# yuanqing-wang/stag

Hardware: AMD Instinct MI355X
Metric: aggregated edges/sec, stochastic-aggregation layer-forward, ogbn-arxiv-shaped CSR (higher is better)
Workload: dtype f32

## Files before the change

stag_amd/csrc/agg_plain.hpp:

```cpp
#pragma once
#include "agg_kernel.hpp"

namespace stag {

#ifndef STAG_PLAIN_WAVES
#define STAG_PLAIN_WAVES 7
#endif

typedef float f32x2_t __attribute__((ext_vector_type(2)));

template <int KIND, bool RELU>
__device__ __forceinline__ void plain_draw4(uint32_t c0, uint32_t c1, const PhiloxKey& key, f32x2_t p0, float p1,
                                            f32x2_t (&w)[2]) {
  uint32_t r[4];
  philox4x32_10(c0, c1, key, r);
  const f32x2_t s = {p1, p1};
  if constexpr (KIND == kNormal) {
    const f32x2_t z01 = f32x2_t{bm_cos(r[1]), bm_sin(r[1])} * bm_radius(r[0]);
    const f32x2_t z23 = f32x2_t{bm_cos(r[3]), bm_sin(r[3])} * bm_radius(r[2]);
    w[0] = __builtin_elementwise_fma(s, z01, p0);
    w[1] = __builtin_elementwise_fma(s, z23, p0);
  } else if constexpr (KIND == kUniform) {
    w[0] = __builtin_elementwise_fma(s, f32x2_t{u01(r[0]), u01(r[1])}, p0);
    w[1] = __builtin_elementwise_fma(s, f32x2_t{u01(r[2]), u01(r[3])}, p0);
  } else {
    w[0] = f32x2_t{u01(r[0]) < p0.x ? 1.0f : 0.0f, u01(r[1]) < p0.y ? 1.0f : 0.0f};
    w[1] = f32x2_t{u01(r[2]) < p0.x ? 1.0f : 0.0f, u01(r[3]) < p0.y ? 1.0f : 0.0f};
  }
  if constexpr (RELU) {
    w[0] = __builtin_elementwise_max(w[0], f32x2_t{0.f, 0.f});
    w[1] = __builtin_elementwise_max(w[1], f32x2_t{0.f, 0.f});
  }
}

template <int KIND, int LPE, bool RELU, class TEAM>
__device__ __forceinline__ void plain_walk(const AggArgs& a, TEAM& T, const int b, const int pend, const int len) {
  const __amdgpu_buffer_rsrc_t ri =
      __builtin_amdgcn_make_buffer_rsrc(const_cast<int32_t*>(a.indices), 0, (int)a.idx_bytes, 0x00020000);
  f32x2_t p0 = {a.p0s, a.p0s};
  asm volatile("" : "+v"(p0));
  const float p1 = KIND == kUniform ? a.p1s - a.p0s : a.p1s;
  const uint32_t pos1 = a.pos_lo + 1u;
  f32x2_t s01 = {0.f, 0.f}, s23 = {0.f, 0.f}, c01 = {0.f, 0.f}, c23 = {0.f, 0.f};
  const int pend1 = pend - 1;
  for (int p = b; p < pend; p += 2) {
    const bool two = p < pend1;
#if STAG_LOAD_PRIO
    __builtin_amdgcn_s_setprio(3);
#endif
    const int u0 = (int)__builtin_amdgcn_raw_buffer_load_b32(ri, p << 2, 0, 0);
    int u1;
    if (two) u1 = (int)__builtin_amdgcn_raw_buffer_load_b32(ri, (p << 2) + 4, 0, 0);
    uint32_t n0 = a.pos_lo + (uint32_t)p, n1 = pos1 + (uint32_t)p;
    asm volatile("" : "+v"(n0));
    asm volatile("" : "+v"(n1));
    u32x4_t x1;
    const u32x4_t x0 = __builtin_amdgcn_raw_buffer_load_b128(T.rx, (int)(__umul24((uint32_t)u0, a.ldxb) + T.koff), 0, STAG_X_AUX);
    if (two) x1 = __builtin_amdgcn_raw_buffer_load_b128(T.rx, (int)(__umul24((uint32_t)u1, a.ldxb) + T.koff), 0, STAG_X_AUX);
#if STAG_LOAD_PRIO
    if (len > STAG_PRIO_MIN_LEN) __builtin_amdgcn_s_setprio(2); else __builtin_amdgcn_s_setprio(0);
#endif
    f32x2_t w0[2], w1[2];
    plain_draw4<KIND, RELU>(n0, T.c1, T.key, p0, p1, w0);
    if (two) plain_draw4<KIND, RELU>(n1, T.c1, T.key, p0, p1, w1);
    const f32x2_t zero = {0.f, 0.f};
    f32x2_t t01 = __builtin_elementwise_fma(w0[0], f32x2_t{__uint_as_float(x0.x), __uint_as_float(x0.y)}, zero);
    f32x2_t t23 = __builtin_elementwise_fma(w0[1], f32x2_t{__uint_as_float(x0.z), __uint_as_float(x0.w)}, zero);
    if (two) {
      asm volatile("" ::: "memory");
      t01 = __builtin_elementwise_fma(w1[0], f32x2_t{__uint_as_float(x1.x), __uint_as_float(x1.y)}, t01);
      t23 = __builtin_elementwise_fma(w1[1], f32x2_t{__uint_as_float(x1.z), __uint_as_float(x1.w)}, t23);
    }
    if (T.kahan) {
      const f32x2_t y01 = t01 - c01, y23 = t23 - c23;
      const f32x2_t n01 = s01 + y01, n23 = s23 + y23;
      c01 = (n01 - s01) - y01; c23 = (n23 - s23) - y23;
      s01 = n01; s23 = n23;
    } else {
      s01 += t01; s23 += t23;
    }
  }
  T.acc[0] = s01.x; T.acc[1] = s01.y; T.acc[2] = s23.x; T.acc[3] = s23.y;
}

template <int KIND, int LPE, bool RELU, bool WALK>
__global__ __launch_bounds__(STAG_BLOCK_THREADS)
__attribute__((amdgpu_waves_per_eu(STAG_PLAIN_WAVES, STAG_PLAIN_WAVES))) void agg_plain_kernel(const AggArgs a_in) {
  static_assert(KIND >= kNormal && (LPE == 32 || LPE == 64), "the plain launch: sampled noise, 32 or 64 lanes per row");
  static_assert(heavy_slots_of<KIND, LPE>() == 1 && mult_of<KIND, LPE>() == 1, "wide shapes walk one slot, one block");
  AggArgs a = a_in;
  if constexpr (WALK) {
    STAG_PIN_S(a.walk.smask); STAG_PIN_S(a.walk.sshift); STAG_PIN_S(a.walk.jh_light);
    STAG_PIN_S(a.walk.sh); STAG_PIN_S(a.walk.lbase); STAG_PIN_S(a.walk.sl); STAG_PIN_S(a.walk.n_total);
  }
  STAG_PIN_S(a.D); STAG_PIN_S(a.units); STAG_PIN_S(a.indptr); STAG_PIN_S(a.indices);
  STAG_PIN_S(a.x); STAG_PIN_S(a.ldxb); STAG_PIN_S(a.x_bytes); STAG_PIN_S(a.idx_bytes);
  STAG_PIN_S(a.p0s); STAG_PIN_S(a.p1s);
  STAG_PIN_S(a.key.k0); STAG_PIN_S(a.key.k1); STAG_PIN_S(a.key.o0); STAG_PIN_S(a.key.o1); STAG_PIN_S(a.key.epoch);
  STAG_PIN_S(a.pos_lo); STAG_PIN_S(a.pos_hi); STAG_PIN_S(a.chunk_base);
  a.nflags = RELU ? kFlagRelu : 0;
  a.in_norm = 0; a.norm_scale_out = nullptr;
  a.src_scale = nullptr;
  a.nidx = nullptr; a.eid = nullptr;
  a.pmode = STAG_PARAM_SCALAR; a.p0 = nullptr; a.p1 = nullptr;
  a.wide = 0;
  __builtin_assume(a.x_bytes != 0);
  __builtin_assume(a.out != nullptr);

  const int c = threadIdx.x % LPE;
  constexpr int TPB = STAG_BLOCK_THREADS / LPE;
  if constexpr (!WALK) {
    const int unit = blockIdx.x * TPB + threadIdx.x / LPE;
    if (unit >= a.n_units) return;
    agg_unit<KIND, LPE, true, 0, 1, 1, 1, false, false, false, RELU ? 3 : 1>(a, unit, c, 0);
  } else {
    const AggArgs::Walk w = a.walk;
    const int stripe = blockIdx.x & w.smask;
    int j = blockIdx.x >> w.sshift;
    int unit0, end;
    if (j < w.jh_light) {
      unit0 = stripe * w.sh + j * TPB;
      end = (stripe + 1) * w.sh;
    } else {
      j -= w.jh_light;
      unit0 = w.lbase + stripe * w.sl + j * TPB;
      end = min(w.lbase + (stripe + 1) * w.sl, w.n_total);
    }
    const int unit = unit0 + threadIdx.x / LPE;
    if (unit >= end) return;
    agg_unit<KIND, LPE, true, 0, 1, 1, 1, false, false, true, RELU ? 3 : 1>(a, unit, c, 0);
  }
}

template <int KIND>
inline void agg_launch_plain_impl(const AggArgs& a, int lpe, bool walk, dim3 grid, hipStream_t s) {
  const dim3 block(STAG_BLOCK_THREADS);
  const bool relu = (a.nflags & kFlagRelu) != 0;
#define STAG_PLAIN_GO(L, R, W) hipLaunchKernelGGL((agg_plain_kernel<KIND, L, R, W>), grid, block, STAG_AGG_LDS_BYTES, s, a)
  if (lpe == 32) {
    if (walk) { if (relu) STAG_PLAIN_GO(32, true, true); else STAG_PLAIN_GO(32, false, true); }
    else      { if (relu) STAG_PLAIN_GO(32, true, false); else STAG_PLAIN_GO(32, false, false); }
  } else {
    if (walk) { if (relu) STAG_PLAIN_GO(64, true, true); else STAG_PLAIN_GO(64, false, true); }
    else      { if (relu) STAG_PLAIN_GO(64, true, false); else STAG_PLAIN_GO(64, false, false); }
  }
#undef STAG_PLAIN_GO
}

}
```

stag_amd/csrc/noise.hpp:

```cpp
#pragma once
#include <hip/hip_runtime.h>
#include <stdint.h>

namespace stag {

constexpr uint32_t kPhiloxM0 = 0xD2511F53u;
constexpr uint32_t kPhiloxM1 = 0xCD9E8D57u;
constexpr uint32_t kPhiloxW0 = 0x9E3779B9u;
constexpr uint32_t kPhiloxW1 = 0xBB67AE85u;

struct PhiloxKey {
  uint32_t k0, k1;
  uint32_t o0, o1;
  const uint64_t* epoch;
};

__device__ __forceinline__ PhiloxKey resolve_epoch(PhiloxKey k) {
  if (k.epoch) {
    const uint64_t o = (((uint64_t)k.o1 << 32) | k.o0) + *k.epoch;
    k.o0 = (uint32_t)o;
    k.o1 = (uint32_t)(o >> 32);
  }
  return k;
}

inline bool counter_space_ok(int64_t pos_base, int64_t n_edges, int64_t chunk_base, int64_t n_chunk) {
  return pos_base >= 0 && n_edges >= 0 && pos_base <= (1ll << 44) - n_edges && chunk_base >= 0 &&
         chunk_base + n_chunk <= (1ll << 20);
}

__device__ __forceinline__ PhiloxKey key_plus(PhiloxKey k, uint64_t d) {
  const uint64_t o = (((uint64_t)k.o1 << 32) | k.o0) + d;
  k.o0 = (uint32_t)o;
  k.o1 = (uint32_t)(o >> 32);
  return k;
}

__device__ __forceinline__ void philox4x32_10(uint32_t c0, uint32_t c1, const PhiloxKey& key,
                                              uint32_t (&r)[4]) {
  uint32_t c2 = key.o0, c3 = key.o1;
  uint32_t k0 = key.k0, k1 = key.k1;
#pragma unroll
  for (int i = 0; i < 10; ++i) {
    const uint64_t p0 = (uint64_t)kPhiloxM0 * c0;
    const uint64_t p1 = (uint64_t)kPhiloxM1 * c2;
    const uint32_t n0 = __builtin_amdgcn_bitop3_b32((uint32_t)(p1 >> 32), c1, k0, 0x96);
    const uint32_t n2 = __builtin_amdgcn_bitop3_b32((uint32_t)(p0 >> 32), c3, k1, 0x96);
    c1 = (uint32_t)p1;
    c3 = (uint32_t)p0;
    c0 = n0;
    c2 = n2;
    k0 += kPhiloxW0;
    k1 += kPhiloxW1;
  }
  r[0] = c0; r[1] = c1; r[2] = c2; r[3] = c3;
}

__device__ __forceinline__ void philox_at(int64_t gpos, uint32_t chunk, const PhiloxKey& key,
                                          uint32_t (&r)[4]) {
  const uint32_t c0 = (uint32_t)((uint64_t)gpos & 0xFFFFFFFFull);
  const uint32_t c1 = chunk | ((uint32_t)((uint64_t)gpos >> 32) << 20);
  philox4x32_10(c0, c1, key, r);
}

__device__ __forceinline__ uint32_t ctr1_of(int64_t gpos, uint32_t chunk) {
  return chunk | ((uint32_t)((uint64_t)gpos >> 32) << 20);
}

__device__ __forceinline__ float f12(uint32_t r) {
  return __uint_as_float((r & 0x007FFFFFu) | 0x3F800000u);
}

__device__ __forceinline__ float u01(uint32_t r) { return f12(r) - 1.0f; }

__device__ __forceinline__ float bm_radius(uint32_t ra) {
  const float u1 = 2.0f - f12(ra);
  return __builtin_amdgcn_sqrtf(-1.3862943611198906f * __builtin_amdgcn_logf(u1));
}
__device__ __forceinline__ float bm_cos(uint32_t rb) { return __builtin_amdgcn_cosf(f12(rb)); }
__device__ __forceinline__ float bm_sin(uint32_t rb) { return __builtin_amdgcn_sinf(f12(rb)); }

__device__ __forceinline__ void box_muller(uint32_t ra, uint32_t rb, float& za, float& zb) {
  const float rad = bm_radius(ra);
  za = rad * bm_cos(rb);
  zb = rad * bm_sin(rb);
}

enum : int { kNone = 0, kExplicit = 1, kNormal = 2, kUniform = 3, kBernoulli = 4 };

enum : int { kFlagRelu = 1, kDerivShift = 1, kDerivMask = 3, kFlagLogScale = 8 };

__device__ __forceinline__ float exp_scale(float log_scale) { return __expf(log_scale); }

template <int KIND>
__device__ __forceinline__ void draw4(uint32_t c0, uint32_t c1, const PhiloxKey& key,
                                      const float (&a)[4], const float (&b)[4], int flags,
                                      float (&w)[4]) {
  static_assert(KIND >= kNormal, "draw4 is for sampled noise");
  uint32_t r[4];
  philox4x32_10(c0, c1, key, r);
  float t[4];
  if constexpr (KIND == kNormal) {
    box_muller(r[0], r[1], t[0], t[1]);
    box_muller(r[2], r[3], t[2], t[3]);
#pragma unroll
    for (int j = 0; j < 4; ++j) w[j] = __builtin_fmaf(b[j], t[j], a[j]);
  } else if constexpr (KIND == kUniform) {
#pragma unroll
    for (int j = 0; j < 4; ++j) { t[j] = u01(r[j]); w[j] = __builtin_fmaf(b[j] - a[j], t[j], a[j]); }
  } else {
#pragma unroll
    for (int j = 0; j < 4; ++j) w[j] = u01(r[j]) < a[j] ? 1.0f : 0.0f;
  }
  const int deriv = (flags >> kDerivShift) & kDerivMask;
  if (deriv == 0) {
    if (flags & kFlagRelu) {
#pragma unroll
      for (int j = 0; j < 4; ++j) w[j] = fmaxf(w[j], 0.0f);
    }
    return;
  }
  if constexpr (KIND != kBernoulli) {
#pragma unroll
    for (int j = 0; j < 4; ++j) {
      const float mask = ((flags & kFlagRelu) && !(w[j] > 0.0f)) ? 0.0f : 1.0f;
      float d;
      if constexpr (KIND == kNormal)
        d = (deriv == 1) ? 1.0f : ((flags & kFlagLogScale) ? t[j] * b[j] : t[j]);
      else d = (deriv == 1) ? 1.0f - t[j] : t[j];
      w[j] = d * mask;
    }
  }
}

template <int KIND>
__device__ __forceinline__ void draw4_grad(uint32_t c0, uint32_t c1, const PhiloxKey& key,
                                           const float (&a)[4], const float (&b)[4], int flags,
                                           float (&w)[4], float (&d0)[4], float (&d1)[4]) {
  static_assert(KIND == kNormal || KIND == kUniform, "only reparameterised draws have derivatives");
  uint32_t r[4];
  philox4x32_10(c0, c1, key, r);
  float t[4];
  if constexpr (KIND == kNormal) {
    box_muller(r[0], r[1], t[0], t[1]);
    box_muller(r[2], r[3], t[2], t[3]);
#pragma unroll
    for (int j = 0; j < 4; ++j) w[j] = __builtin_fmaf(b[j], t[j], a[j]);
  } else {
#pragma unroll
    for (int j = 0; j < 4; ++j) { t[j] = u01(r[j]); w[j] = __builtin_fmaf(b[j] - a[j], t[j], a[j]); }
  }
#pragma unroll
  for (int j = 0; j < 4; ++j) {
    const float mask = ((flags & kFlagRelu) && !(w[j] > 0.0f)) ? 0.0f : 1.0f;
    if (flags & kFlagRelu) w[j] = fmaxf(w[j], 0.0f);
    d0[j] = ((KIND == kNormal) ? 1.0f : 1.0f - t[j]) * mask;
    d1[j] = (KIND == kNormal && (flags & kFlagLogScale)) ? t[j] * b[j] * mask : t[j] * mask;
  }
}

}
```

Measured before the change: 12.70 billion.

## Add wave-uniform walk with scalar index loads and split Philox rounds

Adds a wave-level walk path for 64-lane rows. The edge index and counter are made wave-uniform, so neighbour ids come from scalar constant loads and the gather offset moves to the scalar operand. Philox is split so that the first rounds, which depend only on the edge counter and key, run once per wave on scalar units, and only the remaining rounds run per lane. Kahan compensation and the odd-edge tail become compile-time specialisations. The cost is more code paths and reliance on readfirstlane uniformity assumptions. The path is enabled by default when walk is set and can be switched with an environment variable.

Result: no change. 12.71 billion, median of 3 (+0.1%).

```diff
diff --git a/stag_amd/csrc/agg_plain.hpp b/stag_amd/csrc/agg_plain.hpp
--- a/stag_amd/csrc/agg_plain.hpp
+++ b/stag_amd/csrc/agg_plain.hpp
@@ -10,10 +10,7 @@
 typedef float f32x2_t __attribute__((ext_vector_type(2)));
 
 template <int KIND, bool RELU>
-__device__ __forceinline__ void plain_draw4(uint32_t c0, uint32_t c1, const PhiloxKey& key, f32x2_t p0, float p1,
-                                            f32x2_t (&w)[2]) {
-  uint32_t r[4];
-  philox4x32_10(c0, c1, key, r);
+__device__ __forceinline__ void plain_weights4(const uint32_t (&r)[4], f32x2_t p0, float p1, f32x2_t (&w)[2]) {
   const f32x2_t s = {p1, p1};
   if constexpr (KIND == kNormal) {
     const f32x2_t z01 = f32x2_t{bm_cos(r[1]), bm_sin(r[1])} * bm_radius(r[0]);
@@ -33,8 +30,95 @@
   }
 }
 
+template <int KIND, bool RELU>
+__device__ __forceinline__ void plain_draw4(uint32_t c0, uint32_t c1, const PhiloxKey& key, f32x2_t p0, float p1,
+                                            f32x2_t (&w)[2]) {
+  uint32_t r[4];
+  philox4x32_10(c0, c1, key, r);
+  plain_weights4<KIND, RELU>(r, p0, p1, w);
+}
+
+enum : int32_t { kPlainWaveWalk = 4 };
+
+template <int KIND, bool RELU, class TEAM>
+__device__ __forceinline__ void plain_walk_wave(const AggArgs& a, TEAM& T, const int b_in, const int pend_in, const int len_in) {
+  typedef const int32_t __attribute__((address_space(4))) cid_t;
+  int b = __builtin_amdgcn_readfirstlane(b_in), pend = __builtin_amdgcn_readfirstlane(pend_in);
+  const int len = __builtin_amdgcn_readfirstlane(len_in);
+  asm volatile("" : "+s"(b));
+  asm volatile("" : "+s"(pend));
+  cid_t* const ids = (cid_t*)a.indices;
+  const PhiloxKey key{T.key.k0, T.key.k1, (uint32_t)__builtin_amdgcn_readfirstlane((int)T.key.o0),
+                      (uint32_t)__builtin_amdgcn_readfirstlane((int)T.key.o1), nullptr};
+  f32x2_t p0 = {a.p0s, a.p0s};
+  asm volatile("" : "+v"(p0));
+  const float p1 = KIND == kUniform ? a.p1s - a.p0s : a.p1s;
+  const uint32_t pos1 = a.pos_lo + 1u;
+  f32x2_t s01 = {0.f, 0.f}, s23 = {0.f, 0.f}, c01 = {0.f, 0.f}, c23 = {0.f, 0.f};
+  auto block = [&](const int p, auto two_edges, auto kahan_fold) __attribute__((always_inline)) {
+    constexpr bool TWO = decltype(two_edges)::value, KAHAN = decltype(kahan_fold)::value;
+#if STAG_LOAD_PRIO
+    __builtin_amdgcn_s_setprio(3);
+#endif
+    const int u0 = ids[p];
+    int u1 = 0;
+    if constexpr (TWO) u1 = ids[p + 1];
+    uint32_t n0 = a.pos_lo + (uint32_t)p, n1 = pos1 + (uint32_t)p;
+    asm volatile("" : "+s"(n0));
+    asm volatile("" : "+s"(n1));
+    PhiloxUniform g0, g1;
+    philox4x32_10_uniform(n0, key, g0);
+    if constexpr (TWO) philox4x32_10_uniform(n1, key, g1);
+    u32x4_t x1;
+    const u32x4_t x0 = __builtin_amdgcn_raw_buffer_load_b128(T.rx, (int)T.koff, (int)((uint32_t)u0 * a.ldxb), STAG_X_AUX);
+    if constexpr (TWO) x1 = __builtin_amdgcn_raw_buffer_load_b128(T.rx, (int)T.koff, (int)((uint32_t)u1 * a.ldxb), STAG_X_AUX);
+#if STAG_LOAD_PRIO
+    if (len > STAG_PRIO_MIN_LEN) __builtin_amdgcn_s_setprio(2); else __builtin_amdgcn_s_setprio(0);
+#endif
+    f32x2_t w0[2], w1[2];
+    uint32_t r[4];
+    philox4x32_10_lanes(g0, T.c1, key, r);
+    plain_weights4<KIND, RELU>(r, p0, p1, w0);
+    if constexpr (TWO) {
+      philox4x32_10_lanes(g1, T.c1, key, r);
+      plain_weights4<KIND, RELU>(r, p0, p1, w1);
+    }
+    const f32x2_t zero = {0.f, 0.f};
+    f32x2_t t01 = __builtin_elementwise_fma(w0[0], f32x2_t{__uint_as_float(x0.x), __uint_as_float(x0.y)}, zero);
+    f32x2_t t23 = __builtin_elementwise_fma(w0[1], f32x2_t{__uint_as_float(x0.z), __uint_as_float(x0.w)}, zero);
+    if constexpr (TWO) {
+      t01 = __builtin_elementwise_fma(w1[0], f32x2_t{__uint_as_float(x1.x), __uint_as_float(x1.y)}, t01);
+      t23 = __builtin_elementwise_fma(w1[1], f32x2_t{__uint_as_float(x1.z), __uint_as_float(x1.w)}, t23);
+    }
+    if constexpr (KAHAN) {
+      const f32x2_t y01 = t01 - c01, y23 = t23 - c23;
+      const f32x2_t n01 = s01 + y01, n23 = s23 + y23;
+      c01 = (n01 - s01) - y01; c23 = (n23 - s23) - y23;
+      s01 = n01; s23 = n23;
+    } else {
+      s01 += t01; s23 += t23;
+    }
+  };
+  const int pend1 = pend - 1;
+  int p = b;
+  if (len > kKahanMinLen) {
+    for (; p < pend1; p += 2) block(p, std::true_type{}, std::true_type{});
+    if (p < pend) block(p, std::false_type{}, std::true_type{});
+  } else {
+    for (; p < pend1; p += 2) block(p, std::true_type{}, std::false_type{});
+    if (p < pend) block(p, std::false_type{}, std::false_type{});
+  }
+  T.acc[0] = s01.x; T.acc[1] = s01.y; T.acc[2] = s23.x; T.acc[3] = s23.y;
+}
+
 template <int KIND, int LPE, bool RELU, class TEAM>
 __device__ __forceinline__ void plain_walk(const AggArgs& a, TEAM& T, const int b, const int pend, const int len) {
+  if constexpr (LPE == 64) {
+    if (a.wide & kPlainWaveWalk) {
+      plain_walk_wave<KIND, RELU>(a, T, b, pend, len);
+      return;
+    }
+  }
   const __amdgpu_buffer_rsrc_t ri =
       __builtin_amdgcn_make_buffer_rsrc(const_cast<int32_t*>(a.indices), 0, (int)a.idx_bytes, 0x00020000);
   f32x2_t p0 = {a.p0s, a.p0s};
@@ -103,14 +187,15 @@
   a.src_scale = nullptr;
   a.nidx = nullptr; a.eid = nullptr;
   a.pmode = STAG_PARAM_SCALAR; a.p0 = nullptr; a.p1 = nullptr;
-  a.wide = 0;
+  a.wide = LPE == 64 ? (a_in.wide & kPlainWaveWalk) : 0;
   __builtin_assume(a.x_bytes != 0);
   __builtin_assume(a.out != nullptr);
 
   const int c = threadIdx.x % LPE;
   constexpr int TPB = STAG_BLOCK_THREADS / LPE;
   if constexpr (!WALK) {
-    const int unit = blockIdx.x * TPB + threadIdx.x / LPE;
+    int unit = blockIdx.x * TPB + threadIdx.x / LPE;
+    if constexpr (LPE == 64) unit = __builtin_amdgcn_readfirstlane(unit);
     if (unit >= a.n_units) return;
     agg_unit<KIND, LPE, true, 0, 1, 1, 1, false, false, false, RELU ? 3 : 1>(a, unit, c, 0);
   } else {
@@ -126,14 +211,24 @@
       unit0 = w.lbase + stripe * w.sl + j * TPB;
       end = min(w.lbase + (stripe + 1) * w.sl, w.n_total);
     }
-    const int unit = unit0 + threadIdx.x / LPE;
+    int unit = unit0 + threadIdx.x / LPE;
+    if constexpr (LPE == 64) unit = __builtin_amdgcn_readfirstlane(unit);
     if (unit >= end) return;
     agg_unit<KIND, LPE, true, 0, 1, 1, 1, false, false, true, RELU ? 3 : 1>(a, unit, c, 0);
   }
 }
 
+inline bool wave_walk_enabled(bool walk) {
+  const char* e = getenv("STAG_AGG_WAVE_WALK");
+  if (e && (e[0] == '0' || e[0] == '1') && e[1] == 0) return e[0] == '1';
+  return walk;
+}
+
 template <int KIND>
-inline void agg_launch_plain_impl(const AggArgs& a, int lpe, bool walk, dim3 grid, hipStream_t s) {
+inline void agg_launch_plain_impl(const AggArgs& a_in, int lpe, bool walk, dim3 grid, hipStream_t s) {
+  AggArgs a = a_in;
+  a.wide &= ~kPlainWaveWalk;
+  if (lpe == 64 && wave_walk_enabled(walk)) a.wide |= kPlainWaveWalk;
   const dim3 block(STAG_BLOCK_THREADS);
   const bool relu = (a.nflags & kFlagRelu) != 0;
 #define STAG_PLAIN_GO(L, R, W) hipLaunchKernelGGL((agg_plain_kernel<KIND, L, R, W>), grid, block, STAG_AGG_LDS_BYTES, s, a)
diff --git a/stag_amd/csrc/noise.hpp b/stag_amd/csrc/noise.hpp
--- a/stag_amd/csrc/noise.hpp
+++ b/stag_amd/csrc/noise.hpp
@@ -1,6 +1,12 @@
 #pragma once
+#ifdef STAG_NOISE_HOST
+#include <stdint.h>
+#define __device__
+#define __forceinline__ inline
+#else
 #include <hip/hip_runtime.h>
 #include <stdint.h>
+#endif
 
 namespace stag {
 
@@ -36,6 +42,14 @@
   return k;
 }
 
+__device__ __forceinline__ uint32_t xor3(uint32_t a, uint32_t b, uint32_t c) {
+#ifdef STAG_NOISE_HOST
+  return a ^ b ^ c;
+#else
+  return __builtin_amdgcn_bitop3_b32(a, b, c, 0x96);
+#endif
+}
+
 __device__ __forceinline__ void philox4x32_10(uint32_t c0, uint32_t c1, const PhiloxKey& key,
                                               uint32_t (&r)[4]) {
   uint32_t c2 = key.o0, c3 = key.o1;
@@ -44,8 +58,8 @@
   for (int i = 0; i < 10; ++i) {
     const uint64_t p0 = (uint64_t)kPhiloxM0 * c0;
     const uint64_t p1 = (uint64_t)kPhiloxM1 * c2;
-    const uint32_t n0 = __builtin_amdgcn_bitop3_b32((uint32_t)(p1 >> 32), c1, k0, 0x96);
-    const uint32_t n2 = __builtin_amdgcn_bitop3_b32((uint32_t)(p0 >> 32), c3, k1, 0x96);
+    const uint32_t n0 = xor3((uint32_t)(p1 >> 32), c1, k0);
+    const uint32_t n2 = xor3((uint32_t)(p0 >> 32), c3, k1);
     c1 = (uint32_t)p1;
     c3 = (uint32_t)p0;
     c0 = n0;
@@ -56,6 +70,63 @@
   r[0] = c0; r[1] = c1; r[2] = c2; r[3] = c3;
 }
 
+struct PhiloxUniform {
+  uint32_t a;
+  uint32_t b;
+  uint32_t c;
+  uint32_t d;
+  uint32_t e;
+};
+
+__device__ __forceinline__ void philox4x32_10_uniform(uint32_t c0, const PhiloxKey& key, PhiloxUniform& u) {
+  const uint64_t p0 = (uint64_t)kPhiloxM0 * c0;
+  const uint64_t p1 = (uint64_t)kPhiloxM1 * key.o0;
+  u.a = (uint32_t)(p1 >> 32) ^ key.k0;
+  const uint32_t c2_1 = (uint32_t)(p0 >> 32) ^ key.o1 ^ key.k1;
+  u.b = (uint32_t)p0 ^ (key.k1 + kPhiloxW1);
+  const uint64_t q1 = (uint64_t)kPhiloxM1 * c2_1;
+  const uint32_t c0_2 = (uint32_t)(q1 >> 32) ^ (uint32_t)p1 ^ (key.k0 + kPhiloxW0);
+  u.c = (uint32_t)q1 ^ (key.k0 + 2u * kPhiloxW0);
+  const uint64_t r0 = (uint64_t)kPhiloxM0 * c0_2;
+  u.d = (uint32_t)(r0 >> 32) ^ (key.k1 + 2u * kPhiloxW1);
+  u.e = (uint32_t)r0 ^ (key.k1 + 3u * kPhiloxW1);
+}
+
+__device__ __forceinline__ void philox4x32_10_lanes(const PhiloxUniform& u, uint32_t c1, const PhiloxKey& key,
+                                                    uint32_t (&r)[4]) {
+  const uint64_t q0 = (uint64_t)kPhiloxM0 * (u.a ^ c1);
+  const uint32_t c2_2 = (uint32_t)(q0 >> 32) ^ u.b;
+  const uint64_t r1 = (uint64_t)kPhiloxM1 * c2_2;
+  uint32_t c0 = (uint32_t)(r1 >> 32) ^ u.c;
+  uint32_t c1n = (uint32_t)r1;
+  uint32_t c2 = (uint32_t)q0 ^ u.d;
+  uint32_t k0 = key.k0 + 3u * kPhiloxW0, k1 = key.k1 + 4u * kPhiloxW1;
+  uint32_t c3;
+  {
+    const uint64_t p0 = (uint64_t)kPhiloxM0 * c0;
+    const uint64_t p1 = (uint64_t)kPhiloxM1 * c2;
+    c0 = xor3((uint32_t)(p1 >> 32), c1n, k0);
+    c2 = (uint32_t)(p0 >> 32) ^ u.e;
+    c1n = (uint32_t)p1;
+    c3 = (uint32_t)p0;
+    k0 += kPhiloxW0;
+  }
+#pragma unroll
+  for (int i = 4; i < 10; ++i) {
+    const uint64_t p0 = (uint64_t)kPhiloxM0 * c0;
+    const uint64_t p1 = (uint64_t)kPhiloxM1 * c2;
+    const uint32_t n0 = xor3((uint32_t)(p1 >> 32), c1n, k0);
+    const uint32_t n2 = xor3((uint32_t)(p0 >> 32), c3, k1);
+    c1n = (uint32_t)p1;
+    c3 = (uint32_t)p0;
+    c0 = n0;
+    c2 = n2;
+    k0 += kPhiloxW0;
+    k1 += kPhiloxW1;
+  }
+  r[0] = c0; r[1] = c1n; r[2] = c2; r[3] = c3;
+}
+
 __device__ __forceinline__ void philox_at(int64_t gpos, uint32_t chunk, const PhiloxKey& key,
                                           uint32_t (&r)[4]) {
   const uint32_t c0 = (uint32_t)((uint64_t)gpos & 0xFFFFFFFFull);
@@ -66,6 +137,8 @@
 __device__ __forceinline__ uint32_t ctr1_of(int64_t gpos, uint32_t chunk) {
   return chunk | ((uint32_t)((uint64_t)gpos >> 32) << 20);
 }
+
+#ifndef STAG_NOISE_HOST
 
 __device__ __forceinline__ float f12(uint32_t r) {
   return __uint_as_float((r & 0x007FFFFFu) | 0x3F800000u);
@@ -159,4 +232,6 @@
   }
 }
 
-}
+#endif
+
+}
```
